# hindlet/EPQ_Raytracer

Hardware: AMD Instinct MI355X
Metric: Mrays/s (island.obj 1920x1080 64spp 8-bounce path-trace segments per second) (higher is better)
Workload: dtype f32

## Files before the change

epq_raytracer_amd/_lib.py:

```python
from __future__ import annotations

import ctypes
import os
from ctypes import POINTER, c_char_p, c_float, c_int32, c_int64, c_size_t, c_uint32, c_uint64, c_void_p

import numpy as np

_HERE = os.path.dirname(os.path.abspath(__file__))
LIB_PATH = os.path.join(_HERE, "lib", "libhip_raytrace.so")
DEBUG_LIB_PATH = os.path.join(_HERE, "lib", "libhip_raytrace_debug.so")


MATERIAL_DTYPE = np.dtype([("colour", "<f4", 4), ("emission", "<f4", 4), ("settings", "<f4", 4)])
RAY_DTYPE = np.dtype([("sample_centre", "<f4", 4)])
SPHERE_DTYPE = np.dtype([("centre", "<f4", 3), ("radius", "<f4"), ("material", MATERIAL_DTYPE)])
TRIANGLE_DTYPE = np.dtype([("a", "<f4", 4), ("edge_one", "<f4", 4), ("edge_two", "<f4", 4), ("normal", "<f4", 4)])
MESH_DTYPE = np.dtype([("min_point", "<f4", 3), ("first_index", "<u4"), ("max_point", "<f4", 3), ("len", "<u4"),
                       ("material", MATERIAL_DTYPE)])
assert MATERIAL_DTYPE.itemsize == 48 and RAY_DTYPE.itemsize == 16 and SPHERE_DTYPE.itemsize == 64
assert TRIANGLE_DTYPE.itemsize == 64 and MESH_DTYPE.itemsize == 80


class PushConstants(ctypes.Structure):

# ... 67 lines not shown
class RayQuery(ctypes.Structure):

    _fields_ = [("origin", c_float * 3), ("t_max", c_float), ("direction", c_float * 3), ("reserved", c_uint32)]


class Hit(ctypes.Structure):

    _fields_ = [("t", c_float), ("kind", c_uint32), ("index", c_uint32), ("mesh", c_uint32), ("normal", c_float * 3),
                ("reserved", c_uint32)]


class QueryStats(ctypes.Structure):

    _fields_ = [("method_ran", c_uint32), ("reserved", c_uint32), ("scan_rays", c_uint64), ("tri_tests", c_uint64)]


assert ctypes.sizeof(RayQuery) == 32 and ctypes.sizeof(Hit) == 32 and ctypes.sizeof(QueryStats) == 24
RAY_QUERY_DTYPE = np.dtype([("origin", "<f4", 3), ("t_max", "<f4"), ("direction", "<f4", 3), ("reserved", "<u4")])
HIT_DTYPE = np.dtype([("t", "<f4"), ("kind", "<u4"), ("index", "<u4"), ("mesh", "<u4"), ("normal", "<f4", 3),
                      ("reserved", "<u4")])
assert RAY_QUERY_DTYPE.itemsize == 32 and HIT_DTYPE.itemsize == 32
QUERY_AUTO, QUERY_SCAN, QUERY_BVH, QUERY_PAIRS = 0, 1, 2, 3
QUERY_NAMES = {0: "auto", 1: "scan", 2: "bvh", 3: "pairs"}
HIT_MISS, HIT_SPHERE, HIT_TRIANGLE = 0, 1, 2
HIT_NONE = 0xFFFFFFFF

ABI_VERSION = 6
TILE_LIST_WORDS = 66
HRT_OK = 0
STATUS_NAMES = {0: "HRT_OK", 1: "HRT_ERR_INVALID_ARGUMENT", 2: "HRT_ERR_NO_DEVICE", 3: "HRT_ERR_OUT_OF_MEMORY",
                4: "HRT_ERR_NO_SCENE", 5: "HRT_ERR_HIP", 6: "HRT_ERR_IO", 7: "HRT_ERR_COMM"}
ERR_COMM = 7
MODE_RGBA8, MODE_RGBA32F = 0, 1
IMG_TRACE, IMG_ACCUM = 0, 1
IMG_LOCAL = 0x100
FMT_RGBA8, FMT_RGBA32F = 0, 1
PRESENT_B8G8R8A8, PRESENT_R8G8B8A8 = 0, 1
PRESENT_RING = 8
OPT_KERNEL_VARIANT, OPT_COUNTERS, OPT_SECONDARY_BATCH, OPT_BVH_LEAF_SIZE = 1, 2, 3, 4
OPT_SPLIT, OPT_SPLIT_FACTOR, OPT_PRIORITY, OPT_GRID_CUS, OPT_COOP, OPT_WQ_NODE_CAP, OPT_PROBE = 5, 6, 7, 8, 9, 10, 11
OPT_FRAMES_PER_LAUNCH, OPT_OVERLAP, OPT_BUSY_SPLIT, OPT_BVH_WIDTH, OPT_WQ_NODE_RADIUS = 12, 13, 14, 15, 16
OPT_COMM_TIMEOUT_MS, OPT_DEFER_COMBINE, OPT_FOLD_RECORDS = 17, 18, 19
OPT_SKY_LANE = 20
OPT_WQ_LDS_NODES = 21
DEBUG_OPT_FAIL_ALLOC = 1001
DEBUG_OPT_WQ_TRI_CAP = 1002
DEBUG_OPT_GRAB_RUNS = 1003
DEBUG_OPT_TIMELINE = 1004
DEBUG_OPT_STACK_LIMIT = 1005
COMM_ID_BYTES = 128
COMM_NONE, COMM_RCCL, COMM_RCCL_GROUP, COMM_DEVICE_COPY = 0, 1, 2, 3
KERNEL_AUTO, KERNEL_LITERAL, KERNEL_BRUTE, KERNEL_BRUTE_LDS, KERNEL_BUNDLE, KERNEL_BUNDLE_CULL = 0, 1, 2, 3, 4, 5
KERNEL_BUNDLE_BVH, KERNEL_BUNDLE_CULL_LDS, KERNEL_BUNDLE_BVH_LDS, KERNEL_BUNDLE_WQ = 6, 7, 8, 9
KERNEL_BUNDLE_WQ_L2 = 10
NODE_RADIUS_MARGIN_MILLI = 100


def wq_node_radius(scene_info: dict, option: int = 0) -> bool:
    return option == 2 or (option == 0 and scene_info.get("bvh_margin_milli", 0) > NODE_RADIUS_MARGIN_MILLI)


def kernel_symbol(kernel: int, block: int, diag: bool = False, node_r: bool = False) -> str:
    d = "true" if diag else "false"
    if kernel == 9 and node_r:
        return f"void hrt::trace_bundle_wq_nr<{d}>(hrt::TraceParams)"
    if kernel == 10 and node_r:
        return f"void hrt::trace_bundle_wq_l2_nr<{d}>(hrt::TraceParams)"
    if kernel in (1, 2, 3):
        return "hrt::" + {1: "trace_literal", 2: "trace_brute", 3: "trace_brute_lds"}[kernel] + "(hrt::TraceParams)"
    if kernel == 7:
        return f"void hrt::trace_bundle_cull_lds<{block}, {d}>(hrt::TraceParams)"
    name = {4: "trace_bundle", 5: "trace_bundle_cull", 6: "trace_bundle_bvh", 8: "trace_bundle_bvh_lds",
            9: "trace_bundle_wq", 10: "trace_bundle_wq_l2"}.get(kernel, "?")
    return f"void hrt::{name}<{d}>(hrt::TraceParams)"


KERNEL_NAMES = {0: "auto", 1: "literal", 2: "brute", 3: "brute_lds", 4: "bundle", 5: "bundle_cull", 6: "bundle_bvh",
                7: "bundle_cull_lds", 8: "bundle_bvh_lds", 9: "bundle_wq", 10: "bundle_wq_l2"}
DIAG_NAMES = ("primary_iters", "primary_considered", "primary_survivors", "bounce_iters", "bounce_considered",
              "bounce_survivors", "bounce_lanes", "bvh_visits", "bvh_prim_tests", "bvh_band_tests", "primary_cycles", "bounce_cycles",
              "shade_cycles", "bounce_stage2", "bounce_front", "bvh_trips",
              "bvh_leaf_trips", "band_scan_max", "band_scan_len", "sky_items", "sky_cycles",
              "primary_lanes", "loop_iters", "live_lanes", "wq_steps_16", "wq_steps_32", "wq_steps_48",
              "wq_steps_64", "wq_members")
SCENE_INFO_NAMES = ("bvh_nodes", "bvh_prims", "bvh_irregular", "bvh_never", "bvh_built", "bvh_band_entries",
                    "bvh_sah_milli", "bvh_margin_milli")

EXPORTED_SYMBOLS = (
    "hrt_abi_version", "hrt_build_id", "hrt_debug_build", "hrt_debug_check_guards", "hrt_create", "hrt_destroy", "hrt_set_scene", "hrt_trace", "hrt_accumulate", "hrt_compute_n",
    "hrt_compute_until", "hrt_get_fold_records", "hrt_intersect", "hrt_intersect_primary",
    "hrt_read_image", "hrt_load_accumulator", "hrt_get_layout", "hrt_synchronize", "hrt_get_stats", "hrt_reset_stats", "hrt_set_option",
    "hrt_get_diagnostics", "hrt_get_tile_profile", "hrt_get_scene_info", "hrt_generate_rays", "hrt_read_rays",
    "hrt_import_external_memory", "hrt_release_external_memory",
    "hrt_present", "hrt_accumulate_present", "hrt_present_done", "hrt_present_wait", "hrt_debug_export_memory", "hrt_debug_unmap_memory", "hrt_debug_math_check", "hrt_debug_math_check_rng", "hrt_debug_band_flatten", "hrt_debug_wq_protocol",
    "hrt_debug_timeline", "hrt_debug_band_records", "hrt_debug_tile_costs", "hrt_debug_sky_units",
    "hrt_debug_tile_lists",
    "hrt_stream", "hrt_release_caches", "hrt_last_error", "hrt_comm_unique_id", "hrt_comm_init", "hrt_comm_init_all", "hrt_comm_info",
    "hrt_host_create_rays", "hrt_host_ray_grid", "hrt_host_view_matrix", "hrt_host_transform_meshes",
    "hrt_debug_bvh_build", "hrt_debug_bvh_wq_nodes", "hrt_debug_bvh_wq_nodes_bfs", "hrt_debug_wq_l2_plan",
    "hrt_obj_load", "hrt_obj_num_meshes", "hrt_obj_mesh", "hrt_obj_free",
)


class HrtError(RuntimeError):

    def __init__(self, status: int, where: str, detail: str = ""):
        self.status = status
        super().__init__(f"{where} failed: {STATUS_NAMES.get(status, status)}{': ' + detail if detail else ''}")


_libs = {}


def load(debug: bool = False) -> ctypes.CDLL:
    if debug in _libs:
        return _libs[debug]
    path = DEBUG_LIB_PATH if debug else os.environ.get("HRT_LIB", LIB_PATH)
    if not os.path.exists(path):
        raise RuntimeError(f"{path} is missing: build it with `python -c 'import __graft_entry__ as g; g.build()'`"
                           " or `make -C epq_raytracer_amd/csrc` (no CPU fallback exists)")
    lib = ctypes.CDLL(path)
    lib.hrt_abi_version.restype = c_uint32
    lib.hrt_abi_version.argtypes = []
    if lib.hrt_abi_version() != ABI_VERSION:
        raise RuntimeError(f"{path} implements HRT_ABI_VERSION {lib.hrt_abi_version()}, this binding "
                           f"{ABI_VERSION}: rebuild it (make -C epq_raytracer_amd/csrc)")
    P = c_void_p
    sig = {
        "hrt_abi_version": (c_uint32, []),
        "hrt_debug_build": (c_uint32, []),
        "hrt_build_id": (c_char_p, []),
        "hrt_debug_check_guards": (c_int32, [P, POINTER(c_uint32), POINTER(c_uint32)]),
        "hrt_comm_unique_id": (c_int32, [P]),
        "hrt_comm_init": (c_int32, [P, P, c_uint32, c_uint32]),
        "hrt_comm_init_all": (c_int32, [P, c_uint32]),
        "hrt_comm_info": (c_int32, [P, POINTER(c_uint32), POINTER(c_uint32), POINTER(c_uint32)]),
        "hrt_create": (c_int32, [POINTER(CreateInfo), POINTER(c_void_p)]),
        "hrt_destroy": (None, [P]),
        "hrt_set_scene": (c_int32, [P, P, c_uint32, P, c_uint32, P, c_uint32, P, c_uint32]),
        "hrt_trace": (c_int32, [P, POINTER(PushConstants)]),
        "hrt_accumulate": (c_int32, [P, c_uint32]),
        "hrt_compute_n": (c_int32, [P, POINTER(PushConstants), c_uint32]),
        "hrt_compute_until": (c_int32, [P, POINTER(PushConstants), c_uint32, POINTER(SettleRule), POINTER(c_uint32),
                                        POINTER(c_uint32)]),
        "hrt_get_fold_records": (c_int32, [P, P, c_uint32, POINTER(c_uint32), POINTER(c_uint64)]),
        "hrt_intersect": (c_int32, [P, P, c_uint32, c_uint32, P, POINTER(QueryStats)]),
        "hrt_intersect_primary": (c_int32, [P, POINTER(PushConstants), c_uint32, c_uint32, c_uint32, c_uint32, c_uint32,
                                            P, POINTER(QueryStats)]),
        "hrt_read_image": (c_int32, [P, c_uint32, c_uint32, P, c_size_t]),
        "hrt_load_accumulator": (c_int32, [P, c_uint32, P, c_size_t]),
        "hrt_get_layout": (c_int32, [P, POINTER(Layout)]),
        "hrt_synchronize": (c_int32, [P]),
        "hrt_get_stats": (c_int32, [P, POINTER(Stats)]),
        "hrt_reset_stats": (c_int32, [P]),
        "hrt_get_diagnostics": (c_int32, [P, P, c_uint32]),
        "hrt_get_scene_info": (c_int32, [P, P, c_uint32]),
        "hrt_get_tile_profile": (c_int32, [P, P, c_uint32]),
        "hrt_generate_rays": (c_int32, [P, c_float, c_float, POINTER(c_float), POINTER(c_float)]),
        "hrt_read_rays": (c_int32, [P, P, c_uint32]),
        "hrt_import_external_memory": (c_int32, [P, c_int32, c_uint64, c_uint64, c_uint64, POINTER(c_void_p)]),
        "hrt_release_external_memory": (c_int32, [P, P]),
        "hrt_present": (c_int32, [P, POINTER(PresentInfo), P, c_uint64, POINTER(c_uint64)]),
        "hrt_accumulate_present": (c_int32, [P, c_uint32, POINTER(PresentInfo), P, c_uint64, POINTER(c_uint64)]),
        "hrt_present_done": (c_int32, [P, c_uint64, POINTER(c_uint32)]),
        "hrt_present_wait": (c_int32, [P, c_uint64]),
        "hrt_debug_export_memory": (c_int32, [c_int32, c_uint64, POINTER(c_int32), POINTER(c_void_p),
                                              POINTER(c_uint64)]),
# ... 64 lines not shown
```

epq_raytracer_amd/csrc/hrt_kernels.hip:

```cpp
#include <hip/hip_runtime.h>

#include <algorithm>
#include <mutex>
#include <type_traits>
#include <vector>

#include "hip_raytrace.h"
#include "hrt_bvh.h"
#include "hrt_kernels.h"
#include "hrt_math.h"

namespace hrt {

#ifndef HRT_TIMELINE
#define HRT_TIMELINE 0
#endif
#ifndef HRT_TL_PREPASS
#define HRT_TL_PREPASS 1
#endif



struct Scene {
  const float4* __restrict__ rays;
// ... 251 lines not shown
  return h;
}

template <class PC>
__device__ __forceinline__ f3 environment_light(const PC& pc, f3 d) {
  if (!pc.use_environment_light) return mk(0.0f, 0.0f, 0.0f);
  const float a = 0.5f * (d.y + 1.0f);
  const float oma = 1.0f - a;
  return mk(oma * 1.0f + a * 0.5f, oma * 1.0f + a * 0.7f, oma * 1.0f + a * 1.0f);
}

#ifndef HRT_FUZZ_FAST
#define HRT_FUZZ_FAST 1
#endif
#ifndef HRT_FUZZ_INT
#define HRT_FUZZ_INT 1
#endif
__device__ __forceinline__ f3 adjust_dir(f3 d, f3 n, const hrt_material& mat, bool specular, uint32_t& state) {
  const f3 diffuse_dir = normalize_fl(n + unit_sphere(state));
  const float k = 2.0f * dot(n, d);
  const f3 specular_dir = d - n * k;
  const float a = mat.settings[1] * (float)(int)specular;
  const float oma = 1.0f - a;
#if HRT_FUZZ_FAST
  const float fz = mat.settings[2];
  uint32_t st = state;
  bool fast = a == 0.0f && fz == 0.0f;
#pragma unroll
  for (int c = 0; c < 3; ++c) {
    hash(st);
#if HRT_FUZZ_INT
    fast &= hash(st) - 1u < 0xFFFFFF7Fu;
#else
    const float u = u01(hash(st));
    fast &= u != 0.0f && u != 1.0f;
#endif
  }
  const bool finite_nz = fabsf(diffuse_dir.x) < __builtin_inff() && fabsf(diffuse_dir.y) < __builtin_inff() &&
                         fabsf(diffuse_dir.z) < __builtin_inff() && diffuse_dir.x != 0.0f && diffuse_dir.y != 0.0f &&
                         diffuse_dir.z != 0.0f;
  const bool spec_ok = fabsf(specular_dir.x) < __builtin_inff() && fabsf(specular_dir.y) < __builtin_inff() &&
                       fabsf(specular_dir.z) < __builtin_inff();
  if (fast && finite_nz && spec_ok) {
    state = st;
    return normalize_fl(diffuse_dir);
  }
#endif
  const f3 fuzz = unit_sphere(state) * mat.settings[2];
  const f3 mixed = mk(diffuse_dir.x * oma + specular_dir.x * a, diffuse_dir.y * oma + specular_dir.y * a,
                      diffuse_dir.z * oma + specular_dir.z * a);
  return normalize_fl(mixed + fuzz);
}

struct Path {
  f3 light, colour, pos, dir;
  int bounce;
  bool not_visible;
};

__device__ __forceinline__ bool shade_step(const Scene& sc, const hrt_push_constants& pc, Path& p, const Closest& c,
                                           uint32_t& state) {
  if (c.kind != 0) {
    const HitRecord hit = resolve_hit(sc, c, p.pos, p.dir);
    const hrt_material& m = *hit.mat;
    const bool invis = (m.settings[3] == 1.0f);
    p.pos = adds(hit.pos, (float)(int)invis * 0.001f);
    if (invis && p.not_visible) {
      p.pos = hit.pos + p.dir * 0.001f;
      return false;
    }
    p.not_visible = false;
    const bool is_spec = u01(hash(state)) < m.settings[0];
    p.dir = adjust_dir(p.dir, hit.normal, m, is_spec, state);
    const f3 emitted = ld3(m.emission) * m.emission[3];
    p.light = p.light + emitted * p.colour;
    p.colour = p.colour * ld3(m.colour);
    const float prob = gmax(p.colour.x, gmax(p.colour.y, p.colour.z));
    if (u01(hash(state)) >= prob) return true;
    p.colour = div3(p.colour, prob);
    return false;
  }
  p.light = p.light + environment_light(pc, p.dir);
  return true;
}

__device__ __forceinline__ void store_pixel(const TraceParams& , uint32_t x, uint32_t lr, f3 col,
                                            uint32_t frame = 0) {
  const KArgs K = kargs();
  const size_t idx = (size_t)lr * K->pc.width + x + frame * K->frame_stride;
  uint32_t* img8 = K->img8;
  float4* img32 = K->img32;
  if (img8) img8[idx] = unorm8(col.x) | (unorm8(col.y) << 8) | (unorm8(col.z) << 16) | (255u << 24);
  if (img32) img32[idx] = make_float4(col.x, col.y, col.z, 1.0f);
}

__device__ __forceinline__ void wave_counters(uint32_t segs, uint32_t tests, unsigned long long& s,
                                              unsigned long long& t, uint32_t& mx) {
  s = segs;
  t = tests;
  mx = segs;
#pragma unroll
  for (int off = 32; off > 0; off >>= 1) {
    s += __shfl_xor(s, off, 64);
    t += __shfl_xor(t, off, 64);
    mx = max(mx, (uint32_t)__shfl_xor((int)mx, off, 64));
  }
}
__device__ __forceinline__ void add_counters(const TraceParams& , unsigned long long s, unsigned long long t,
                                             unsigned long long mx) {
  unsigned long long* counters = kargs()->counters;
  if (counters && (threadIdx.x & 63) == 0) {
    atomicAdd(&counters[0], s);
    atomicAdd(&counters[1], t);
    atomicAdd(&counters[2], mx);
  }
}
__device__ __forceinline__ void flush_counters(const TraceParams& P, uint32_t segs, uint32_t tests) {
  if (!kargs()->counters) return;
  unsigned long long s, t;
  uint32_t mx;
  wave_counters(segs, tests, s, t, mx);
  add_counters(P, s, t, mx);
}

__device__ __forceinline__ void lane_pixel(const TraceParams& P, uint32_t& x, uint32_t& lr) {
  const uint32_t wave = threadIdx.x >> 6, lane = threadIdx.x & 63;
  x = blockIdx.x * 16 + (wave & 1) * 8 + (lane & 7);
  lr = blockIdx.y * 16 + (wave >> 1) * 8 + (lane >> 3);
}

__global__ __launch_bounds__(256) void trace_literal(TraceParams P) {
  const Scene sc{P.rays, P.spheres, P.tris, P.meshes, P.tri_nhat};
  const hrt_push_constants& pc = P.pc;
  uint32_t x, lr;
  lane_pixel(P, x, lr);
  const uint32_t y = global_row(lr, P);
  uint32_t segs = 0, tests = 0;
  if (x < pc.width && lr < P.local_rows && y < pc.height) {
    const uint32_t id = x + y * pc.width;
    f3 colour = mk(0.0f, 0.0f, 0.0f);
    uint32_t state = pc.rng_offset * 719393u + id;
    const float4 rc = sc.rays[id];
    const f3 centre = mk(rc.x, rc.y, rc.z);
    const f3 root = mk(pc.cam_pos[0], pc.cam_pos[1], pc.cam_pos[2]);
    for (int s = 0; s < pc.num_samples; ++s) {
      const f3 dir = get_ray_dir(pc, centre, state);
      Path p{mk(0.0f, 0.0f, 0.0f), mk(1.0f, 1.0f, 1.0f), root, normalize(dir), 0, true};
      for (int i = 0; i <= pc.max_bounces; ++i) {
        const Closest c = world_hit_literal(sc, pc, p.pos, p.dir, tests);
        ++segs;
        if (shade_step(sc, pc, p, c, state)) break;
      }
      colour = colour + p.light * p.colour;
    }
    colour = div3(colour, (float)pc.num_samples);
    store_pixel(P, x, lr, colour);
  }
  flush_counters(P, segs, tests);
}

constexpr float kTiny = 8.673617379884035e-19f;
constexpr float kOnePlus = 1.0000152587890625f;
constexpr float kTMin = 0.000999f;

struct TriPre {
  float num_t, num_u, num_v, det;
// ... 85 lines not shown

template <class Src>
__device__ __forceinline__ void trace_fused(const TraceParams& P, const Src& src, uint32_t x, uint32_t lr) {
  const Scene sc{P.rays, P.spheres, P.tris, P.meshes, P.tri_nhat};
  const hrt_push_constants& pc = P.pc;
  const uint32_t y = global_row(lr, P);
  uint32_t segs = 0, tests = 0;
  const bool active = x < pc.width && lr < P.local_rows && y < pc.height;
  if (active) {
    const uint32_t id = x + y * pc.width;
    f3 colour = mk(0.0f, 0.0f, 0.0f);
    uint32_t state = pc.rng_offset * 719393u + id;
    const float4 rc = sc.rays[id];
    const f3 centre = mk(rc.x, rc.y, rc.z);
    const f3 root = mk(pc.cam_pos[0], pc.cam_pos[1], pc.cam_pos[2]);
    int sample = 0;
    Path p;
    p.bounce = pc.max_bounces + 1;
    while (true) {
      if (p.bounce > pc.max_bounces) {
        if (sample >= pc.num_samples) break;
        ++sample;
        const f3 dir = get_ray_dir(pc, centre, state);
        p = Path{mk(0.0f, 0.0f, 0.0f), mk(1.0f, 1.0f, 1.0f), root, normalize(dir), 0, true};
      }
      const Closest c = world_hit_brute(sc, src, pc, p.pos, p.dir, tests);
      ++segs;
      const bool ended = shade_step(sc, pc, p, c, state);
      ++p.bounce;
      if (ended || p.bounce > pc.max_bounces) {
        colour = colour + p.light * p.colour;
        p.bounce = pc.max_bounces + 1;
      }
    }
    colour = div3(colour, (float)pc.num_samples);
    store_pixel(P, x, lr, colour);
  }
  flush_counters(P, segs, tests);
}

__global__ __launch_bounds__(256) void trace_brute(TraceParams P) {
  uint32_t x, lr;
  lane_pixel(P, x, lr);
  trace_fused(P, GlobalTris{reinterpret_cast<const float4*>(P.tris)}, x, lr);
}

extern __shared__ float4 lds_tris[];
__global__ __launch_bounds__(1024) void trace_brute_lds(TraceParams P) {
  const uint32_t n = P.n_tris;
  for (uint32_t k = threadIdx.x; k < 3 * n; k += blockDim.x) {
    const uint32_t i = k / 3, part = k - 3 * i;
    const hrt_triangle& t = P.tris[i];
    float4 v;
    if (part == 0) v = make_float4(t.a[0], t.a[1], t.a[2], t.normal[0]);
    else if (part == 1) v = make_float4(t.normal[1], t.normal[2], t.edge_one[0], t.edge_one[1]);
    else v = make_float4(t.edge_one[2], t.edge_two[0], t.edge_two[1], t.edge_two[2]);
    lds_tris[k] = v;
  }
  __syncthreads();
  const uint32_t wave = threadIdx.x >> 6, lane = threadIdx.x & 63;
  const uint32_t x = blockIdx.x * 32 + (wave & 3) * 8 + (lane & 7);
  const uint32_t lr = blockIdx.y * 32 + (wave >> 2) * 8 + (lane >> 3);
  trace_fused(P, LdsTris{lds_tris}, x, lr);
}

struct Bundle {
  f3 a;
  float c_lo, c_hi, s_hi;
};

struct Diag {
  uint32_t prim_iters = 0, prim_considered = 0, prim_survivors = 0;
  uint32_t sec_iters = 0, sec_considered = 0, sec_survivors = 0, sec_lanes = 0;
  uint32_t bvh_visits = 0, bvh_prims = 0, bvh_band = 0;
  uint64_t cyc_prim = 0, cyc_sec = 0, cyc_shade = 0;
  uint32_t sec_stage2 = 0, sec_front = 0;
  uint32_t bvh_trips = 0, bvh_leaf_trips = 0;
  uint32_t band_max = 0, band_len = 0;
  uint32_t sky_items = 0;
  uint64_t cyc_sky = 0;
  uint32_t prim_lanes = 0, loop_iters = 0, live_lanes = 0;
  uint32_t wq_fill[4] = {0, 0, 0, 0};
  uint32_t wq_members = 0;
};

__device__ __forceinline__ float wave_min_all(float v) {
#pragma unroll
  for (int off = 32; off > 0; off >>= 1) v = fminf(v, __shfl_xor(v, off, 64));
  return v;
}
__device__ __forceinline__ uint32_t wave_max_u(uint32_t v) {
#pragma unroll
  for (int off = 32; off > 0; off >>= 1) v = max(v, (uint32_t)__shfl_xor((int)v, off, 64));
  return v;
}
__device__ __forceinline__ float wave_max_all(float v) {
#pragma unroll
  for (int off = 32; off > 0; off >>= 1) v = fmaxf(v, __shfl_xor(v, off, 64));
  return v;
}

__device__ __forceinline__ Bundle make_bundle(bool sel, f3 d) {
  const int lead = __builtin_ctzll(__ballot(sel));
  Bundle b;
  b.a = mk(lane_read(d.x, (uint32_t)lead), lane_read(d.y, (uint32_t)lead), lane_read(d.z, (uint32_t)lead));
  const float lam = sel ? dot(d, b.a) : 3.0f;
  b.c_lo = wave_min_all(lam) - 1e-5f;
  b.c_hi = 1.00001f;
  b.s_hi = (b.c_lo > 0.0f) ? __builtin_sqrtf(fmaxf(0.0f, 1.00002f - b.c_lo * b.c_lo)) * 1.00001f + 1e-6f : 1.00001f;
  return b;
}

__device__ __forceinline__ float lin_lower(float ga, float gn, const Bundle& b) {
  return fminf(b.c_lo * ga, b.c_hi * ga) - b.s_hi * gn;
}
__device__ __forceinline__ float lin_upper(float ga, float gn, const Bundle& b) {
  return fmaxf(b.c_lo * ga, b.c_hi * ga) + b.s_hi * gn;
}

__device__ __forceinline__ void spheres_first(const Scene& sc, const hrt_push_constants& pc, bool sel, f3 o, f3 d,
                                              Closest& c) {
  if (!sel) return;
  c = Closest{kFltMax, 0, 0u, 0u};
  for (int i = 0; i < pc.num_spheres; ++i) {
    const float t = sphere_dist(sc.spheres[i], o, d);
    if (t > 0.001f && t < c.t) c = Closest{t, 1, (uint32_t)i, 0u};
  }
}

typedef __attribute__((address_space(4))) const float kfloat;
__device__ __forceinline__ const kfloat* to_const(const float4* p) {
  return (const kfloat*)(const __attribute__((address_space(4))) void*)(p);
}
__device__ __forceinline__ float4 ldk(const kfloat* p, uint32_t i) {
  return make_float4(p[4 * i], p[4 * i + 1], p[4 * i + 2], p[4 * i + 3]);
}

__device__ __forceinline__ void primary_exact_rec(const float4& A, const float4& B, const float4& C, float dn, f3 d,
                                                  uint32_t m, Closest& c, float& best_k) {
  TriPre q;
  q.num_t = A.w;
  const f3 dao = cross(mk(A.x, A.y, A.z), d);
  q.num_u = dot(mk(C.x, C.y, C.z), dao);
  q.num_v = dot(mk(B.x, B.y, B.z), dao);
  q.det = -dn;
  q.cand = (dn < 0.0f) & !pre_reject(q, best_k);
  if (__builtin_expect(__any(q.cand), 0)) {
    if (q.cand) tri_exact(q, __builtin_bit_cast(uint32_t, B.w), m, c, best_k);
  }
}
__device__ __forceinline__ void primary_exact(const kfloat* ct, uint32_t k, float dn, f3 d, uint32_t m, Closest& c,
                                              float& best_k) {
  primary_exact_rec(ldk(ct, 4 * k), ldk(ct, 4 * k + 1), ldk(ct, 4 * k + 2), dn, d, m, c, best_k);
}
typedef float kf16 __attribute__((ext_vector_type(16)));
typedef __attribute__((address_space(4))) const kf16 kf16c;
__device__ __forceinline__ kf16 ld_rec(const kfloat* ct, uint32_t k) { return *(kf16c*)(ct + 16 * (size_t)k); }

constexpr uint32_t kTileCapVgpr = 64;
constexpr uint32_t kTileCapLds = 1024;

struct TileList {
  uint32_t v;
  uint32_t* lds;
  uint32_t n;
  bool ok;
// ... 1160 lines not shown
    for (; s + HRT_SKY_UNROLL <= ns; s += HRT_SKY_UNROLL) {
#pragma unroll
      for (int u = 0; u < HRT_SKY_UNROLL; ++u) sky_segment<false>(K, tl, active, centre, state, colour, t);
    }
    for (; s < ns; ++s) sky_segment<false>(K, tl, active, centre, state, colour, t);
  }
  if (active) {
    segs += ns > 0 ? (uint32_t)ns : 0u;
    tests += t;
  }
}

#ifndef HRT_BOUNCE_PRIO
#define HRT_BOUNCE_PRIO 1
#endif
enum BounceMode {
  kBounceBrute = 0,
  kBounceCull = 1,
  kBounceBvh = 2,
  kBounceWq = 3,
  kBounceWqR = 4,
  kBounceWqL2 = 5,
  kBounceWqL2R = 6
};
constexpr bool is_wq(int b) { return b == kBounceWq || b == kBounceWqR || b == kBounceWqL2 || b == kBounceWqL2R; }
constexpr bool is_wq_node_r(int b) { return b == kBounceWqR || b == kBounceWqL2R; }

#ifndef HRT_PIXEL_POOL
#define HRT_PIXEL_POOL 1
#endif
template <int Bounce, bool D, class CullSrc, class BvhSrc = BvhGlobal>
__device__ __forceinline__ void trace_fused_split(const TraceParams& P, uint32_t x, uint32_t lr, const CullSrc& csrc,
                                                  const BvhSrc& bsrc, uint32_t* list_lds, Coop& co,
                                                  uint32_t frame = 0, uint32_t nrun = 1) {
  const Scene sc{P.rays, P.spheres, P.tris, P.meshes, P.tri_nhat};
  const hrt_push_constants& pc = P.pc;
  const GlobalTris src{reinterpret_cast<const float4*>(P.tris)};
  uint32_t y = global_row(lr, P);
  uint32_t segs = 0, tests = 0;
  const bool active = x < pc.width && lr < kargs()->local_rows && y < pc.height;
  uint32_t id = active ? x + y * pc.width : 0u;
  const uint64_t tile_t0 = (D && P.tile_cycles) ? __builtin_readcyclecounter() : 0;
  f3 colour = mk(0.0f, 0.0f, 0.0f);
  uint32_t state = (pc.rng_offset + frame) * 719393u + id;
  f3 centre = mk(0.0f, 0.0f, 0.0f);
  if (active) {
    const float4 rc = kargs()->rays[id];
    centre = mk(rc.x, rc.y, rc.z);
  }
#if HRT_TL_PREPASS
  TileList tl;
  if (co.cache_tile != 0xFFFFFFFFu && !list_lds) {
    const uint32_t* rec = kargs()->tl_cache + (size_t)co.cache_tile * kTlRecWords;
    const uint32_t lane = threadIdx.x & 63;
    tl.v = rec[lane];
    tl.tsum = rec[64 + lane];
    tl.lds = nullptr;
    tl.n = __builtin_amdgcn_readfirstlane(rec[128]);
    tl.ok = __builtin_amdgcn_readfirstlane(rec[129]) != 0u;
    tl.aabb = (unsigned long long)__builtin_amdgcn_readfirstlane(rec[130]) |
              ((unsigned long long)__builtin_amdgcn_readfirstlane(rec[131]) << 32);
    tl.aabb_ok = __builtin_amdgcn_readfirstlane(rec[132]) != 0u;
  } else {
    tl = build_tile_list(P, active, centre, list_lds);
  }
  if constexpr (is_wq(Bounce)) {
    if (bsrc.capped) {
      tl.n = __builtin_amdgcn_readfirstlane(tl.n);
      tl.aabb = (unsigned long long)__builtin_amdgcn_readfirstlane((uint32_t)tl.aabb) |
                ((unsigned long long)__builtin_amdgcn_readfirstlane((uint32_t)(tl.aabb >> 32)) << 32);
    }
  }
#else
  const TileList tl = build_tile_list(P, active, centre, list_lds);
#endif
#if HRT_TIMELINE
  co.t_setup = __builtin_amdgcn_s_memrealtime();
  co.t_sky = tl.ok && tl.n == 0u && pc.num_spheres == 0;
#endif
  const uint32_t sec_thresh = max(1u, (kargs()->sec_batch * (uint32_t)__popcll(__ballot(active)) + 63u) / 64u);
  int sample = 0;
  Path p;
  p.bounce = pc.max_bounces + 1;
  bool done = !active;
  Diag dg;
  uint32_t fr = 0;
  const bool pool = HRT_PIXEL_POOL && nrun > 1u && __all(active);
  uint32_t pool_next = 64u;
  if (HRT_SKY_LOOP && tl.ok && tl.n == 0u && pc.num_spheres == 0) {
    const uint64_t s0 = (D && P.diag) ? __builtin_readcyclecounter() : 0;
    for (;; ++fr) {
      sky_samples(tl, active, centre, state, colour, segs, tests);
      if (fr + 1u >= nrun) break;
      if (active) store_pixel(P, x, lr, div3(colour, (float)pc.num_samples), frame + fr);
      colour = mk(0.0f, 0.0f, 0.0f);
      state = (pc.rng_offset + frame + fr + 1u) * 719393u + id;
    }
    const uint32_t ns = pc.num_samples > 0 ? (uint32_t)pc.num_samples : 0u;
    if (co.w == 0) co.work += (2u + 3u * ns) * nrun;
    if (D && P.diag) {
      dg.prim_iters += ns * nrun;
      dg.sky_items += nrun;
      dg.cyc_sky += __builtin_readcyclecounter() - s0;
    }
    done = true;
  }
  while (__any(!done)) {
    while (pool) {
      const bool need = !done && p.bounce > pc.max_bounces && sample >= pc.num_samples;
      const unsigned long long nb = __ballot(need);
      if (!nb) break;
      {
        if (need) store_pixel(P, x, lr, div3(colour, (float)pc.num_samples), frame + fr);
        const uint32_t idx = pool_next + lanes_below(nb);
        pool_next += (uint32_t)__popcll(nb);
        if (need) {
          if (idx < 64u * nrun) {
            const uint32_t px = idx & 63u;
            fr = idx >> 6;
            x = (x & ~7u) + (px & 7u);
            lr = (lr & ~7u) + (px >> 3);
            y = global_row(lr, P);
            id = x + y * pc.width;
            const float4 rc = kargs()->rays[id];
            centre = mk(rc.x, rc.y, rc.z);
            colour = mk(0.0f, 0.0f, 0.0f);
            sample = 0;
            state = (pc.rng_offset + frame + fr) * 719393u + id;
          } else {
            done = true;
            fr = nrun;
          }
        }
      }
    }
    if (!done && p.bounce > pc.max_bounces) {
      while (!pool && sample >= pc.num_samples && fr + 1u < nrun) {
        store_pixel(P, x, lr, div3(colour, (float)pc.num_samples), frame + fr);
        ++fr;
        colour = mk(0.0f, 0.0f, 0.0f);
        sample = 0;
        state = (pc.rng_offset + frame + fr) * 719393u + id;
      }
      if (sample >= pc.num_samples) {
        done = true;
      } else {
        ++sample;
        const KArgs K = kargs();
        const f3 dir = get_ray_dir(K->pc, centre, state);
        p = Path{mk(0.0f, 0.0f, 0.0f), mk(1.0f, 1.0f, 1.0f), mk(K->pc.cam_pos[0], K->pc.cam_pos[1], K->pc.cam_pos[2]),
                 normalize_fl(dir), 0, true};
      }
    }
    const bool ready = !done && p.bounce == 0;
    const bool waiting = !done && p.bounce != 0;
    const uint32_t nwait = (uint32_t)__popcll(__ballot(waiting));
    const bool prim = ready;
    const bool any_prim = __any(prim);
    const bool run_sec = nwait > 0 && (nwait >= sec_thresh || !any_prim);
    const bool sec = waiting && run_sec;
    Closest c{kFltMax, 0, 0u, 0u};
    uint64_t t0 = 0, t1 = 0, t2 = 0;
    if (D && P.diag) {
      dg.prim_iters += any_prim ? 1u : 0u;
      dg.sec_iters += run_sec ? 1u : 0u;
      dg.sec_lanes += run_sec ? nwait : 0u;
      dg.prim_lanes += (uint32_t)__popcll(__ballot(prim));
      dg.loop_iters += 1u;
      dg.live_lanes += (uint32_t)__popcll(__ballot(!done));
      t0 = __builtin_readcyclecounter();
    }
    if (co.w == 0) co.work += 2u + (any_prim ? 1u + (tl.ok ? tl.n : 64u) : 0u);
    if (any_prim) {
      if (tl.ok) {
        const uint32_t tested = world_hit_tile(kscene(), P, tl, prim, p.pos, p.dir, tests, c);
        if (D && P.diag) {
          dg.prim_considered += tl.n;
          dg.prim_survivors += tested;
        }
      } else {
        world_hit_bundle<D>(sc, P, prim, p.pos, p.dir, tests, c, dg);
      }
    }
    if (D && P.diag) t1 = __builtin_readcyclecounter();
    if (run_sec) {
      if (HRT_BOUNCE_PRIO && !co.hot) __builtin_amdgcn_s_setprio(HRT_BOUNCE_PRIO);
      if constexpr (is_wq(Bounce)) {
        world_hit_bounce_wq<D, is_wq_node_r(Bounce)>(kscene(), P, bsrc, sec, p.pos, p.dir, tests,
                                                     c, dg);
      } else if constexpr (Bounce == kBounceBvh) {
        world_hit_bounce_bvh<D>(sc, P, bsrc, sec, p.pos, p.dir, tests, c, dg);
      } else if constexpr (Bounce == kBounceCull) {
        world_hit_bounce_cull<D>(sc, P, csrc, sec, p.pos, p.dir, tests, c, dg, co);
      } else {
        if (sec) c = world_hit_brute(sc, src, pc, p.pos, p.dir, tests);
      }
    }
    if (HRT_BOUNCE_PRIO && run_sec && !co.hot) __builtin_amdgcn_s_setprio(0);
    if (D && P.diag) t2 = __builtin_readcyclecounter();
    if (prim || sec) {
      ++segs;
      const bool ended = shade_step(kscene(), pc, p, c, state);
      ++p.bounce;
      if (ended || p.bounce > pc.max_bounces) {
        colour = colour + p.light * p.colour;
        p.bounce = pc.max_bounces + 1;
      }
    }
    if (D && P.diag) {
      const uint64_t t3 = __builtin_readcyclecounter();
      dg.cyc_prim += t1 - t0;
      dg.cyc_sec += t2 - t1;
      dg.cyc_shade += t3 - t2;
    }
  }
  if (co.w != 0) return;
  if (active && fr < nrun) {
    colour = div3(colour, (float)pc.num_samples);
    store_pixel(P, x, lr, colour, frame + fr);
  }
  if (co.defer) {
    unsigned long long s, t;
    uint32_t mx;
    wave_counters(segs, tests, s, t, mx);
    co.acc_s += s;
    co.acc_t += t;
    co.acc_m += mx;
  } else {
    flush_counters(P, segs, tests);
  }
  if (D && P.tile_cycles && (threadIdx.x & 63) == 0) {
    const uint32_t tiles_x = (pc.width + 7) / 8;
    unsigned long long* rec = P.tile_cycles + 4 * ((lr / 8) * tiles_x + x / 8);
    atomicMax(&rec[0], (unsigned long long)(__builtin_readcyclecounter() - tile_t0));
    atomicAdd(&rec[1], (unsigned long long)dg.sec_iters |
                           (is_wq(Bounce) ? (unsigned long long)dg.bvh_trips << 32 : 0ull));
    if (Bounce != kBounceBvh && !is_wq(Bounce)) atomicAdd(&rec[2], (unsigned long long)dg.sec_survivors);
    atomicAdd(&rec[3], (unsigned long long)dg.cyc_sec);
  }
  if (D && P.tile_cycles && (Bounce == kBounceBvh || is_wq(Bounce)) && active) {
    const uint32_t tiles_x = (pc.width + 7) / 8;
    atomicAdd(P.tile_cycles + 4 * ((lr / 8) * tiles_x + x / 8) + 2,
              (unsigned long long)dg.bvh_visits + ((unsigned long long)(dg.bvh_prims + dg.bvh_band) << 32));
  }
  if (D && P.diag && (threadIdx.x & 63) == 0) {
    atomicAdd(&P.diag[10], (unsigned long long)dg.cyc_prim);
    atomicAdd(&P.diag[11], (unsigned long long)dg.cyc_sec);
    atomicAdd(&P.diag[12], (unsigned long long)dg.cyc_shade);
    atomicAdd(&P.diag[13], (unsigned long long)dg.sec_stage2);
    atomicAdd(&P.diag[14], (unsigned long long)dg.sec_front);
    atomicAdd(&P.diag[15], (unsigned long long)dg.bvh_trips);
    atomicAdd(&P.diag[16], (unsigned long long)dg.bvh_leaf_trips);
    atomicAdd(&P.diag[17], (unsigned long long)dg.band_max);
    atomicAdd(&P.diag[0], (unsigned long long)dg.prim_iters);
    atomicAdd(&P.diag[1], (unsigned long long)dg.prim_considered);
    atomicAdd(&P.diag[2], (unsigned long long)dg.prim_survivors);
    atomicAdd(&P.diag[3], (unsigned long long)dg.sec_iters);
    atomicAdd(&P.diag[4], (unsigned long long)dg.sec_considered);
    atomicAdd(&P.diag[5], (unsigned long long)dg.sec_survivors);
    atomicAdd(&P.diag[6], (unsigned long long)dg.sec_lanes);
    if (dg.sky_items) {
      atomicAdd(&P.diag[19], (unsigned long long)dg.sky_items);
      atomicAdd(&P.diag[20], (unsigned long long)dg.cyc_sky);
    }
    atomicAdd(&P.diag[21], (unsigned long long)dg.prim_lanes);
    atomicAdd(&P.diag[22], (unsigned long long)dg.loop_iters);
    atomicAdd(&P.diag[23], (unsigned long long)dg.live_lanes);
    if (is_wq(Bounce)) {
#pragma unroll
      for (int b = 0; b < 4; ++b) atomicAdd(&P.diag[24 + b], (unsigned long long)dg.wq_fill[b]);
    }
  }
  if (D && P.diag && is_wq(Bounce) && dg.wq_members) atomicAdd(&P.diag[28], (unsigned long long)dg.wq_members);
  if (D && P.diag && (Bounce == kBounceBvh || is_wq(Bounce))) {
    atomicAdd(&P.diag[7], (unsigned long long)dg.bvh_visits);
    atomicAdd(&P.diag[8], (unsigned long long)dg.bvh_prims);
    atomicAdd(&P.diag[9], (unsigned long long)dg.bvh_band);
    atomicAdd(&P.diag[18], (unsigned long long)dg.band_len);
  }
}

template <bool D>
__global__ __launch_bounds__(256) void trace_bundle(TraceParams P) {
  __shared__ uint32_t lists[4 * kTileCapLds];
  uint32_t x, lr;
  lane_pixel(P, x, lr);
  const float4* T = reinterpret_cast<const float4*>(P.tris);
  Coop solo{0u, 1u, nullptr, 0u, 0u};
  trace_fused_split<kBounceBrute, D>(P, x, lr, CullGlobal{T, to_const(T)}, BvhGlobal{},
                                     lists + (threadIdx.x >> 6) * kTileCapLds, solo);
}

#ifndef HRT_CULL_WAVES
#define HRT_CULL_WAVES 1
#endif
template <bool D>
__global__ __launch_bounds__(256) __attribute__((amdgpu_waves_per_eu(HRT_CULL_WAVES))) void trace_bundle_cull(
    TraceParams P) {
  __shared__ uint32_t lists[4 * kTileCapLds];
  uint32_t x, lr;
  lane_pixel(P, x, lr);
  const float4* T = reinterpret_cast<const float4*>(P.tris);
  Coop solo{0u, 1u, nullptr, 0u, 0u};
  trace_fused_split<kBounceCull, D>(P, x, lr, CullGlobal{T, to_const(T)}, BvhGlobal{},
                                    lists + (threadIdx.x >> 6) * kTileCapLds, solo);
}

template <bool D>
__global__ __launch_bounds__(256) void trace_bundle_bvh(TraceParams P) {
  __shared__ uint32_t lists[4 * kTileCapLds];
  uint32_t x, lr;
  lane_pixel(P, x, lr);
  const float4* T = reinterpret_cast<const float4*>(P.tris);
  Coop solo{0u, 1u, nullptr, 0u, 0u};
  trace_fused_split<kBounceBvh, D>(P, x, lr, CullGlobal{T, to_const(T)}, BvhGlobal{P.bvh_nodes, P.bvh_prims},
                                   lists + (threadIdx.x >> 6) * kTileCapLds, solo);
}


__device__ __forceinline__ void stage_tris(const TraceParams& P, float4* dst, uint32_t block) {
  const uint32_t n = P.n_tris;
  for (uint32_t k = threadIdx.x; k < 3 * n; k += block) {
    const uint32_t i = k / 3, part = k - 3 * i;
    const hrt_triangle& t = P.tris[i];
    float4 v;
    if (part == 0) v = make_float4(t.a[0], t.a[1], t.a[2], t.normal[0]);
    else if (part == 1) v = make_float4(t.normal[1], t.normal[2], t.edge_one[0], t.edge_one[1]);
    else v = make_float4(t.edge_one[2], t.edge_two[0], t.edge_two[1], t.edge_two[2]);
    dst[k] = v;
  }
}

constexpr uint32_t kItemTileMask = (1u << 22) - 1u;
constexpr uint32_t kSchedSky = 1000, kSchedQueue = 1002;
static_assert(kSchedQueue + 2 <= kSchedWords && kSchedQueue % 2 == 0, "sched buffer");
template <int BLOCK, bool CoopOk, bool Sky = false, class Body>
__device__ __forceinline__ void tile_loop(const TraceParams& P, unsigned long long* ex, uint32_t* s_item, Body&& body) {
  const uint32_t lane = threadIdx.x & 63;
  const uint32_t tiles_x = (P.pc.width + 7) / 8, tiles = tiles_x * ((P.local_rows + 7) / 8);
  const uint32_t nf = P.n_frames > 1 ? P.n_frames : 1u;
  const uint32_t n = (P.items ? P.sched[1] : tiles) * nf;
  uint32_t first = 0;
  if (CoopOk && P.items && P.coop) {
    const uint32_t H = P.sched[2] * nf;
    first = H;
    Coop co{threadIdx.x >> 6, (uint32_t)BLOCK / 64, ex, 0u, 0u};
    uint32_t prev_tile = 0xFFFFFFFFu, prev_cost = 0;
    for (;;) {
      if (lane == 0) {
        if (prev_tile != 0xFFFFFFFFu) {
          atomicAdd(&P.tile_cost[prev_tile], prev_cost);
          atomicAdd(reinterpret_cast<unsigned long long*>(P.sched + 6), (unsigned long long)prev_cost);
        }
        if (threadIdx.x == 0) *s_item = atomicAdd(&P.sched[5], 1u);
      }
      __syncthreads();
// ... 950 lines not shown
```

include/hip_raytrace.h:

```cpp
#ifndef HIP_RAYTRACE_H
#define HIP_RAYTRACE_H

#include <stddef.h>
#include <stdint.h>

#ifdef __cplusplus
extern "C" {
#endif

#define HRT_ABI_VERSION 6u

typedef enum hrt_status {
  HRT_OK = 0,
  HRT_ERR_INVALID_ARGUMENT = 1,
  HRT_ERR_NO_DEVICE = 2,
  HRT_ERR_OUT_OF_MEMORY = 3,
  HRT_ERR_NO_SCENE = 4,
  HRT_ERR_HIP = 5,
  HRT_ERR_IO = 6,
  HRT_ERR_COMM = 7
} hrt_status;


typedef struct hrt_material {
// ... 183 lines not shown
                  "hrt_ray_query");
HRT_STATIC_ASSERT(sizeof(hrt_hit) == 32 && offsetof(hrt_hit, kind) == 4 && offsetof(hrt_hit, index) == 8 &&
                      offsetof(hrt_hit, mesh) == 12 && offsetof(hrt_hit, normal) == 16 && offsetof(hrt_hit, reserved) == 28,
                  "hrt_hit");
HRT_STATIC_ASSERT(sizeof(hrt_query_stats) == 24 && offsetof(hrt_query_stats, scan_rays) == 8 &&
                      offsetof(hrt_query_stats, tri_tests) == 16,
                  "hrt_query_stats");

typedef struct hrt_context hrt_context;

typedef enum hrt_kernel {
  HRT_KERNEL_AUTO = 0,
  HRT_KERNEL_LITERAL = 1,
  HRT_KERNEL_BRUTE = 2,
  HRT_KERNEL_BRUTE_LDS = 3,
  HRT_KERNEL_BUNDLE = 4,
  HRT_KERNEL_BUNDLE_CULL = 5,
  HRT_KERNEL_BUNDLE_BVH = 6,
  HRT_KERNEL_BUNDLE_CULL_LDS = 7,
  HRT_KERNEL_BUNDLE_BVH_LDS = 8,
  HRT_KERNEL_BUNDLE_WQ = 9,
  HRT_KERNEL_BUNDLE_WQ_L2 = 10,
} hrt_kernel;

typedef enum hrt_option {
  HRT_OPT_KERNEL_VARIANT = 1,
  HRT_OPT_COUNTERS = 2,
  HRT_OPT_SECONDARY_BATCH = 3,
  HRT_OPT_BVH_LEAF_SIZE = 4,
  HRT_OPT_SPLIT = 5,
  HRT_OPT_SPLIT_FACTOR = 6,
  HRT_OPT_PRIORITY = 7,
  HRT_OPT_GRID_CUS = 8,
  HRT_OPT_COOP = 9,
  HRT_OPT_WQ_NODE_CAP = 10,
  HRT_OPT_PROBE = 11,
  HRT_OPT_FRAMES_PER_LAUNCH = 12,
  HRT_OPT_OVERLAP = 13,
  HRT_OPT_BUSY_SPLIT = 14,
  HRT_OPT_BVH_WIDTH = 15,
  HRT_OPT_WQ_NODE_RADIUS = 16,
  HRT_OPT_COMM_TIMEOUT_MS = 17,
  HRT_OPT_DEFER_COMBINE = 18,
  HRT_OPT_FOLD_RECORDS = 19,
  HRT_OPT_SKY_LANE = 20,
  HRT_OPT_WQ_LDS_NODES = 21,
  HRT_DEBUG_OPT_FAIL_ALLOC = 1001,
  HRT_DEBUG_OPT_WQ_TRI_CAP = 1002,
  HRT_DEBUG_OPT_GRAB_RUNS = 1003,
  HRT_DEBUG_OPT_TIMELINE = 1004,
  HRT_DEBUG_OPT_STACK_LIMIT = 1005
} hrt_option;

typedef enum hrt_diag {
  HRT_DIAG_PRIMARY_ITERS = 0,
  HRT_DIAG_PRIMARY_CONSIDERED = 1,
  HRT_DIAG_PRIMARY_SURVIVORS = 2,
  HRT_DIAG_BOUNCE_ITERS = 3,
  HRT_DIAG_BOUNCE_CONSIDERED = 4,
  HRT_DIAG_BOUNCE_SURVIVORS = 5,
  HRT_DIAG_BOUNCE_LANES = 6,
  HRT_DIAG_BVH_VISITS = 7,
  HRT_DIAG_BVH_PRIM_TESTS = 8,
  HRT_DIAG_BVH_BAND_TESTS = 9,
  HRT_DIAG_PRIMARY_CYCLES = 10,
  HRT_DIAG_BOUNCE_CYCLES = 11,
  HRT_DIAG_SHADE_CYCLES = 12,
  HRT_DIAG_BOUNCE_STAGE2 = 13,
  HRT_DIAG_BOUNCE_FRONT = 14,
  HRT_DIAG_BVH_TRIPS = 15,
  HRT_DIAG_BVH_LEAF_TRIPS = 16,
  HRT_DIAG_BAND_SCAN_MAX = 17,
  HRT_DIAG_BAND_SCAN_LEN = 18,
  HRT_DIAG_SKY_ITEMS = 19,
  HRT_DIAG_SKY_CYCLES = 20,
  HRT_DIAG_PRIMARY_LANES = 21,
  HRT_DIAG_LOOP_ITERS = 22,
  HRT_DIAG_LIVE_LANES = 23,
  HRT_DIAG_WQ_STEPS_16 = 24,
  HRT_DIAG_WQ_STEPS_32 = 25,
  HRT_DIAG_WQ_STEPS_48 = 26,
  HRT_DIAG_WQ_STEPS_64 = 27,
  HRT_DIAG_WQ_MEMBERS = 28,
  HRT_NUM_DIAG = 29
} hrt_diag;

typedef enum hrt_scene_info {
  HRT_SCENE_BVH_NODES = 0,
  HRT_SCENE_BVH_PRIMS = 1,
  HRT_SCENE_BVH_IRREGULAR = 2,
  HRT_SCENE_BVH_NEVER = 3,
  HRT_SCENE_BVH_BUILT = 4,
  HRT_SCENE_BVH_BAND_ENTRIES = 5,
  HRT_SCENE_BVH_SAH_MILLI = 6,
  HRT_SCENE_BVH_MARGIN_MILLI = 7,
  HRT_NUM_SCENE_INFO = 8
} hrt_scene_info;

uint32_t hrt_abi_version(void);
const char* hrt_build_id(void);
uint32_t hrt_debug_build(void);
hrt_status hrt_debug_check_guards(hrt_context* ctx, uint32_t* buffers, uint32_t* corrupted);

hrt_status hrt_create(const hrt_create_info* info, hrt_context** out_ctx);
void hrt_destroy(hrt_context* ctx);

hrt_status hrt_set_scene(hrt_context* ctx, const hrt_ray* rays, uint32_t n_rays, const hrt_sphere* spheres,
                         uint32_t n_spheres, const hrt_triangle* tris, uint32_t n_tris, const hrt_mesh* meshes,
                         uint32_t n_meshes);

hrt_status hrt_trace(hrt_context* ctx, const hrt_push_constants* pc);

hrt_status hrt_accumulate(hrt_context* ctx, uint32_t frame);

hrt_status hrt_compute_n(hrt_context* ctx, const hrt_push_constants* pc, uint32_t n);

hrt_status hrt_intersect(hrt_context* ctx, const hrt_ray_query* rays, uint32_t n, uint32_t method, hrt_hit* hits,
                         hrt_query_stats* stats);

hrt_status hrt_intersect_primary(hrt_context* ctx, const hrt_push_constants* pc, uint32_t x0, uint32_t y0,
                                 uint32_t w, uint32_t h, uint32_t method, hrt_hit* hits, hrt_query_stats* stats);

hrt_status hrt_get_fold_records(hrt_context* ctx, hrt_fold_record* out, uint32_t cap, uint32_t* count,
                                uint64_t* total);

hrt_status hrt_compute_until(hrt_context* ctx, const hrt_push_constants* pc, uint32_t max_frames,
                             const hrt_settle_rule* rule, uint32_t* frames_done, uint32_t* settled);

hrt_status hrt_read_image(hrt_context* ctx, uint32_t image_id, uint32_t fmt, void* dst, size_t bytes);

hrt_status hrt_load_accumulator(hrt_context* ctx, uint32_t fmt, const void* src, size_t bytes);

#define HRT_COMM_ID_BYTES 128
typedef enum hrt_comm_transport {
  HRT_COMM_NONE = 0,
  HRT_COMM_RCCL = 1,
  HRT_COMM_RCCL_GROUP = 2,
  HRT_COMM_DEVICE_COPY = 3
} hrt_comm_transport;
hrt_status hrt_comm_unique_id(uint8_t id[HRT_COMM_ID_BYTES]);
hrt_status hrt_comm_init(hrt_context* ctx, const uint8_t id[HRT_COMM_ID_BYTES], uint32_t rank, uint32_t world);
hrt_status hrt_comm_init_all(hrt_context* const* ctxs, uint32_t n);
hrt_status hrt_comm_info(const hrt_context* ctx, uint32_t* rank, uint32_t* world, uint32_t* transport);

hrt_status hrt_get_layout(const hrt_context* ctx, hrt_layout* out);
hrt_status hrt_synchronize(hrt_context* ctx);
hrt_status hrt_get_stats(hrt_context* ctx, hrt_stats* out);
hrt_status hrt_reset_stats(hrt_context* ctx);
hrt_status hrt_get_diagnostics(hrt_context* ctx, uint64_t* out, uint32_t count);
hrt_status hrt_get_tile_profile(hrt_context* ctx, uint64_t* out, uint32_t count);
hrt_status hrt_get_scene_info(hrt_context* ctx, uint32_t* out, uint32_t count);

hrt_status hrt_generate_rays(hrt_context* ctx, float camera_focal_length, float viewport_height, const float up[3],
                             float* default_jitter);
hrt_status hrt_read_rays(hrt_context* ctx, hrt_ray* out, uint32_t n);

hrt_status hrt_import_external_memory(hrt_context* ctx, int fd, uint64_t size, uint64_t offset, uint64_t bytes,
                                      void** dev_ptr);
hrt_status hrt_release_external_memory(hrt_context* ctx, void* dev_ptr);

hrt_status hrt_present(hrt_context* ctx, const hrt_present_info* info, void* dst, uint64_t dst_bytes,
                       uint64_t* ticket);
hrt_status hrt_accumulate_present(hrt_context* ctx, uint32_t frame, const hrt_present_info* info, void* dst,
                                  uint64_t dst_bytes, uint64_t* ticket);
hrt_status hrt_present_done(hrt_context* ctx, uint64_t ticket, uint32_t* done);
hrt_status hrt_present_wait(hrt_context* ctx, uint64_t ticket);
hrt_status hrt_debug_export_memory(int device, uint64_t bytes, int* fd, void** ptr, uint64_t* size);
// ... 30 lines not shown
```

Measured before the change: 99750.

## Defer bounce direction sampling until the next secondary trace step

Splits the shading step into shade_hit and shade_dir. shade_hit handles emission, throughput and Russian roulette and records a pending hit. shade_dir computes the normal and the new scattered direction just before the next bounce trace. Paths killed by roulette or on the last bounce no longer pay for normal fetch and direction sampling, and the direction work runs in the secondary phase where lanes are grouped. It also changes the RNG stream order (a fixed 12-hash skip) and adds a dir_lanes diagnostic counter. This risks extra register pressure from the pending state carried across loop iterations.

After: 101,100, median of 6. 1.01x the previous value.

```diff
diff --git a/epq_raytracer_amd/_lib.py b/epq_raytracer_amd/_lib.py
--- a/epq_raytracer_amd/_lib.py
+++ b/epq_raytracer_amd/_lib.py
@@ -173,7 +173,7 @@
               "shade_cycles", "bounce_stage2", "bounce_front", "bvh_trips",
               "bvh_leaf_trips", "band_scan_max", "band_scan_len", "sky_items", "sky_cycles",
               "primary_lanes", "loop_iters", "live_lanes", "wq_steps_16", "wq_steps_32", "wq_steps_48",
-              "wq_steps_64", "wq_members")
+              "wq_steps_64", "wq_members", "dir_lanes")
 SCENE_INFO_NAMES = ("bvh_nodes", "bvh_prims", "bvh_irregular", "bvh_never", "bvh_built", "bvh_band_entries",
                     "bvh_sah_milli", "bvh_margin_milli")
 
diff --git a/epq_raytracer_amd/csrc/hrt_kernels.hip b/epq_raytracer_amd/csrc/hrt_kernels.hip
--- a/epq_raytracer_amd/csrc/hrt_kernels.hip
+++ b/epq_raytracer_amd/csrc/hrt_kernels.hip
@@ -357,6 +357,95 @@
   }
   p.light = p.light + environment_light(pc, p.dir);
   return true;
+}
+
+#ifndef HRT_SHADE_PREDRAW
+#define HRT_SHADE_PREDRAW 0
+#endif
+template <bool Packed>
+struct Pending {
+  uint32_t id = 0;
+  uint32_t mesh = 0;
+  bool sphere = false;
+#if HRT_SHADE_PREDRAW
+  uint32_t st = 0;
+#endif
+  __device__ __forceinline__ uint32_t tri() const { return Packed ? (id - 1u) & 0x3FFFFFFu : id - 1u; }
+  __device__ __forceinline__ uint32_t mesh_of() const { return Packed ? (id - 1u) >> 26 : mesh; }
+};
+
+template <bool Packed>
+__device__ __forceinline__ bool shade_hit(const Scene& sc, const hrt_push_constants& pc, Path& p, const Closest& c,
+                                          uint32_t& state, bool last, Pending<Packed>& pd) {
+  if (c.kind != 0) {
+    const bool sph = c.kind == 1;
+    const f3 hpos = ray_at(p.pos, p.dir, c.t);
+    const hrt_material& m = sph ? sc.spheres[c.idx].material : sc.meshes[c.mesh].material;
+    const bool invis = (m.settings[3] == 1.0f);
+    p.pos = adds(hpos, (float)(int)invis * 0.001f);
+    if (invis && p.not_visible) {
+      p.pos = hpos + p.dir * 0.001f;
+      return false;
+    }
+    p.not_visible = false;
+    uint32_t st = state;
+    const uint32_t s1 = hash(st);
+#pragma unroll
+    for (int k = 0; k < 12; ++k) hash(st);
+    const f3 emitted = ld3(m.emission) * m.emission[3];
+    p.light = p.light + emitted * p.colour;
+    p.colour = p.colour * ld3(m.colour);
+    const float prob = gmax(p.colour.x, gmax(p.colour.y, p.colour.z));
+    if (u01(hash(st)) >= prob) {
+      state = st;
+      return true;
+    }
+    p.colour = div3(p.colour, prob);
+    if (last) {
+      state = st;
+      return false;
+    }
+    if (sph) p.pos = hpos;
+    pd.id = (Packed && !sph ? (c.mesh << 26) | c.idx : c.idx) + 1u;
+    pd.mesh = c.mesh;
+    pd.sphere = sph;
+#if HRT_SHADE_PREDRAW
+    pd.st = s1;
+    state = st;
+#else
+    (void)s1;
+#endif
+    return false;
+  }
+  p.light = p.light + environment_light(pc, p.dir);
+  return true;
+}
+
+template <bool Packed>
+__device__ __forceinline__ void shade_dir(const Scene& sc, Path& p, uint32_t& state, Pending<Packed>& pd) {
+  f3 n;
+  const hrt_material* mat;
+  if (pd.sphere) {
+    const hrt_sphere& s = sc.spheres[pd.id - 1u];
+    n = normalize(p.pos - ld3(s.centre));
+    mat = &s.material;
+    p.pos = adds(p.pos, (float)(int)(s.material.settings[3] == 1.0f) * 0.001f);
+  } else {
+    const float4 nh = sc.nhat[pd.tri()];
+    n = mk(nh.x, nh.y, nh.z);
+    mat = &sc.meshes[pd.mesh_of()].material;
+  }
+  const hrt_material& m = *mat;
+#if HRT_SHADE_PREDRAW
+  uint32_t st = pd.st;
+  const bool is_spec = u01(st) < m.settings[0];
+  p.dir = adjust_dir(p.dir, n, m, is_spec, st);
+#else
+  const bool is_spec = u01(hash(state)) < m.settings[0];
+  p.dir = adjust_dir(p.dir, n, m, is_spec, state);
+  hash(state);
+#endif
+  pd.id = 0u;
 }
 
 __device__ __forceinline__ void store_pixel(const TraceParams& , uint32_t x, uint32_t lr, f3 col,
@@ -608,6 +697,7 @@
   uint32_t prim_lanes = 0, loop_iters = 0, live_lanes = 0;
   uint32_t wq_fill[4] = {0, 0, 0, 0};
   uint32_t wq_members = 0;
+  uint32_t dir_lanes = 0;
 };
 
 __device__ __forceinline__ float wave_min_all(float v) {
@@ -1934,6 +2024,7 @@
   int sample = 0;
   Path p;
   p.bounce = pc.max_bounces + 1;
+  Pending<is_wq(Bounce)> pd;
   bool done = !active;
   Diag dg;
   uint32_t fr = 0;
@@ -2012,7 +2103,7 @@
     const bool run_sec = nwait > 0 && (nwait >= sec_thresh || !any_prim);
     const bool sec = waiting && run_sec;
     Closest c{kFltMax, 0, 0u, 0u};
-    uint64_t t0 = 0, t1 = 0, t2 = 0;
+    uint64_t t0 = 0, t1 = 0, t2 = 0, tb = 0;
     if (D && P.diag) {
       dg.prim_iters += any_prim ? 1u : 0u;
       dg.sec_iters += run_sec ? 1u : 0u;
@@ -2036,6 +2127,10 @@
     }
     if (D && P.diag) t1 = __builtin_readcyclecounter();
     if (run_sec) {
+      const bool owed = sec && pd.id != 0u;
+      if (D && P.diag) dg.dir_lanes += (uint32_t)__popcll(__ballot(owed));
+      if (owed) shade_dir(kscene(), p, state, pd);
+      if (D && P.diag) tb = __builtin_readcyclecounter() - t1;
       if (HRT_BOUNCE_PRIO && !co.hot) __builtin_amdgcn_s_setprio(HRT_BOUNCE_PRIO);
       if constexpr (is_wq(Bounce)) {
         world_hit_bounce_wq<D, is_wq_node_r(Bounce)>(kscene(), P, bsrc, sec, p.pos, p.dir, tests,
@@ -2052,7 +2147,7 @@
     if (D && P.diag) t2 = __builtin_readcyclecounter();
     if (prim || sec) {
       ++segs;
-      const bool ended = shade_step(kscene(), pc, p, c, state);
+      const bool ended = shade_hit(kscene(), pc, p, c, state, p.bounce >= pc.max_bounces, pd);
       ++p.bounce;
       if (ended || p.bounce > pc.max_bounces) {
         colour = colour + p.light * p.colour;
@@ -2062,8 +2157,8 @@
     if (D && P.diag) {
       const uint64_t t3 = __builtin_readcyclecounter();
       dg.cyc_prim += t1 - t0;
-      dg.cyc_sec += t2 - t1;
-      dg.cyc_shade += t3 - t2;
+      dg.cyc_sec += t2 - t1 - tb;
+      dg.cyc_shade += t3 - t2 + tb;
     }
   }
   if (co.w != 0) return;
@@ -2124,6 +2219,7 @@
     }
   }
   if (D && P.diag && is_wq(Bounce) && dg.wq_members) atomicAdd(&P.diag[28], (unsigned long long)dg.wq_members);
+  if (D && P.diag && dg.dir_lanes && (threadIdx.x & 63) == 0) atomicAdd(&P.diag[29], (unsigned long long)dg.dir_lanes);
   if (D && P.diag && (Bounce == kBounceBvh || is_wq(Bounce))) {
     atomicAdd(&P.diag[7], (unsigned long long)dg.bvh_visits);
     atomicAdd(&P.diag[8], (unsigned long long)dg.bvh_prims);
diff --git a/include/hip_raytrace.h b/include/hip_raytrace.h
--- a/include/hip_raytrace.h
+++ b/include/hip_raytrace.h
@@ -289,7 +289,8 @@
   HRT_DIAG_WQ_STEPS_48 = 26,
   HRT_DIAG_WQ_STEPS_64 = 27,
   HRT_DIAG_WQ_MEMBERS = 28,
-  HRT_NUM_DIAG = 29
+  HRT_DIAG_DIR_LANES = 29,
+  HRT_NUM_DIAG = 30
 } hrt_diag;
 
 typedef enum hrt_scene_info {
```
